# simochen/flowtrack.pytorch

Hardware: AMD Instinct MI355X
Metric: pose crops/sec (ResNet-50 + 3-deconv head, 256x192) (higher is better)
Workload: dtype fp16; 1 GPU; ResNet-50 pose head fp16, batch 64 x 256x192 synthetic crops per GPU (BASELINE.json configs[1]); per_gpu_batch=64, resident_batches=4, parallelism=dp1: batch sharded, one process per GPU

## Files before the change

### flowtrack/pytorch_amd/_lib.py

```python
from __future__ import annotations

import ctypes
import os
from ctypes import POINTER, c_char_p, c_double, c_float, c_int, c_int32, c_uint64, c_void_p

HERE = os.path.dirname(os.path.abspath(__file__))
LIB_PATH = os.environ.get("FT_LIB_PATH") or os.path.join(HERE, "libflowtrack_hip.so")

FT_OK = 0
FT_ERR_INVALID_ARG = 1
FT_ERR_UNSUPPORTED = 2
FT_F16, FT_F32 = 0, 1
FT_ACT_NONE, FT_ACT_RELU, FT_ACT_LEAKY = 0, 1, 2
FT_LAYOUT_NHWC, FT_LAYOUT_NCHW_F32 = 0, 1
FT_RGB_MEAN_SPLITS = 64
FT_BNK_Y_FULL, FT_BNK_Y_EVEN, FT_BNK_Y_NONE = 0, 1, 2


class FlowtrackHipError(RuntimeError):
    pass


class ConvDesc(ctypes.Structure):

# ... 43 lines not shown
    "ft_stream_synchronize": (c_int, [c_void_p]),
    "ft_memcpy_async": (c_int, [c_void_p, c_void_p, ctypes.c_size_t, c_void_p]),
    "ft_conv_pack_geometry": (c_int, [POINTER(ConvDesc), POINTER(ConvGeometry)]),
    "ft_conv_tile_candidates": (c_int, [POINTER(ConvDesc), POINTER(c_int), c_int]),
    "ft_conv_workspace_bytes": (ctypes.c_size_t, [POINTER(ConvDesc)]),
    "ft_conv2d_fwd_ws": (c_int, [POINTER(ConvDesc), c_void_p, c_void_p, c_void_p, c_void_p, c_void_p, c_void_p, c_void_p,
                                 ctypes.c_size_t, c_void_p]),
    "ft_conv_tap_source": (c_int, [POINTER(ConvDesc), c_int, c_int, c_int, POINTER(c_int), POINTER(c_int)]),
    "ft_conv2d_fwd": (c_int, [POINTER(ConvDesc), c_void_p, c_void_p, c_void_p, c_void_p, c_void_p,
                              c_void_p, c_void_p]),
    "ft_conv_flops": (c_double, [POINTER(ConvDesc)]),
    "ft_conv_direct_supported": (c_int, [POINTER(ConvDesc)]),
    "ft_conv_direct_stream_id": (c_int, [POINTER(ConvDesc)]),
    "ft_conv_direct_weight_bytes": (ctypes.c_longlong, [POINTER(ConvDesc)]),
    "ft_conv_direct_pack": (c_int, [POINTER(ConvDesc), c_void_p, c_int, c_int, c_void_p, c_void_p]),
    "ft_conv_direct_fwd": (c_int, [POINTER(ConvDesc), c_void_p, c_void_p, c_void_p, c_void_p, c_void_p, c_void_p, c_void_p]),
    "ft_bottleneck_supported": (c_int, [POINTER(BottleneckDesc)]),
    "ft_bottleneck_fwd": (c_int, [POINTER(BottleneckDesc), c_void_p, c_void_p, c_void_p, c_void_p, c_void_p, c_void_p, c_void_p]),
    "ft_bottleneck_flops": (c_double, [POINTER(BottleneckDesc)]),
    "ft_bottleneck_exit_supported": (c_int, [POINTER(BottleneckDesc), c_int, c_int, c_int, c_int]),
    "ft_bottleneck_exit_weight_bytes": (ctypes.c_longlong, [POINTER(BottleneckDesc), c_int]),
    "ft_bottleneck_exit_pack": (c_int, [POINTER(BottleneckDesc), c_int, c_void_p, c_int, c_int, c_void_p, c_void_p]),
    "ft_bottleneck_exit_fwd": (c_int, [POINTER(BottleneckDesc), c_void_p, c_void_p, c_void_p, c_void_p, c_void_p, c_void_p, c_int, c_int,
                                       c_void_p, c_void_p, c_void_p, c_void_p, c_int, c_int, c_void_p]),
    "ft_bottleneck_rstat_supported": (c_int, [POINTER(BottleneckDesc)]),
    "ft_bottleneck_rstat_weight_bytes": (ctypes.c_longlong, []),
    "ft_bottleneck_rstat_fwd": (c_int, [POINTER(BottleneckDesc), c_void_p, c_void_p, c_void_p, c_void_p]),
    "ft_bottleneck_stream_supported": (c_int, [POINTER(BottleneckDesc)]),
    "ft_bottleneck_stream_folds": (c_int, [POINTER(BottleneckDesc)]),
    "ft_bottleneck_stream_layout": (c_int, [POINTER(BottleneckDesc)]),
    "ft_bottleneck_stream_weight_bytes": (ctypes.c_longlong, [POINTER(BottleneckDesc)]),
    "ft_bottleneck_stream_pack": (c_int, [POINTER(BottleneckDesc), c_void_p, c_void_p, c_void_p, c_void_p, c_void_p]),
    "ft_bottleneck_stream_fwd": (c_int, [POINTER(BottleneckDesc), c_void_p, c_void_p, c_void_p, c_void_p, c_void_p]),
    "ft_pack_nchw_to_nhwc": (c_int, [c_void_p, c_void_p] + [c_int] * 8 + [c_void_p]),
    "ft_unpack_nhwc_to_nchw": (c_int, [c_void_p, c_void_p, c_int, c_int, c_int, c_int, c_int, c_int, c_int,
                                       c_void_p]),
    "ft_maxpool3x3s2_fwd": (c_int, [c_void_p, c_void_p, c_int, c_int, c_int, c_int, c_int, c_void_p]),
    "ft_bn_batch_stats": (c_int, [c_void_p, c_int, c_int, c_int, c_int, c_int, c_int, c_void_p, c_void_p, c_void_p, c_void_p]),
    "ft_heatmap_max_preds": (c_int, [c_void_p, c_int, c_int, c_int, c_int, c_int, c_void_p, c_void_p, c_void_p,
                                     c_void_p]),
    "ft_heatmap_keypoint_rows": (c_int, [c_void_p, c_int, c_int, c_int, c_int, c_int, c_void_p, c_void_p, c_void_p]),
    "ft_heatmap_min_margin": (c_int, [c_void_p, c_int, c_int, c_int, c_int, c_void_p, c_void_p]),
    "ft_heatmap_argmax_screen": (c_int, [c_void_p, c_int, c_int, c_int, c_int, c_float, c_void_p, c_void_p, c_void_p]),
    "ft_flow_rgb_mean": (c_int, [c_void_p, c_int, c_int, c_int, c_void_p, c_void_p, c_void_p]),
    "ft_flow_pack_pair": (c_int, [c_void_p, c_void_p, c_float, c_void_p] + [c_int] * 7 + [c_void_p]),
    "ft_flow_mean_pack_pair_state_words": (ctypes.c_longlong, [c_int, c_int, c_int]),
    "ft_flow_pack_pair_sums_chunks": (ctypes.c_longlong, [c_int]),
    "ft_conv_shift_nstride_supported": (c_int, [POINTER(ConvDesc)]),
    "ft_flow_pack_pair_sums": (c_int, [c_void_p, c_float, c_void_p] + [c_int] * 6 + [c_void_p, c_void_p]),
    "ft_flow_mean_fold": (c_int, [c_void_p, c_float, c_void_p] + [c_int] * 6 + [c_void_p, c_void_p, c_void_p, c_int, c_void_p, c_void_p,
                                  c_void_p]),
    "ft_flow_mean_pack_pair": (c_int, [c_void_p, c_float, c_void_p, c_int, c_int, c_void_p, c_int, c_int] + [c_int] * 4
                               + [c_void_p, c_void_p, c_void_p]),
    "ft_upsample_bilinear4x": (c_int, [c_void_p, c_void_p, c_int, c_int, c_int, c_int, c_float, c_void_p]),
    "ft_correlation_out_shape": (c_int, [c_int] * 8 + [POINTER(c_int)] * 3),
    "ft_correlation_fwd": (c_int, [c_void_p, c_void_p, c_void_p] + [c_int] * 10 + [c_void_p]),
    "ft_correlation_nhwc_fwd": (c_int, [c_void_p, c_void_p, c_void_p] + [c_int] * 10 + [c_float, c_int, c_void_p]),
    "ft_resample2d_fwd": (c_int, [c_void_p, c_void_p, c_void_p, c_int, c_int, c_int, c_int, c_void_p]),
    "ft_channelnorm_fwd": (c_int, [c_void_p, c_void_p, c_int, c_int, c_int, c_int, c_void_p]),
    "ft_correlation_bwd": (c_int, [c_void_p] * 5 + [c_int] * 10 + [c_void_p]),
    "ft_resample2d_bwd": (c_int, [c_void_p] * 5 + [c_int] * 4 + [c_void_p]),
    "ft_channelnorm_bwd": (c_int, [c_void_p] * 4 + [c_int] * 4 + [c_void_p]),
    "ft_upsample_nearest4x": (c_int, [c_void_p, c_void_p, c_int, c_int, c_int, c_int, c_float, c_void_p]),
    "ft_flow_fusion_concat": (c_int, [c_void_p, c_void_p, c_void_p, c_void_p] + [c_int] * 8 + [c_void_p]),
    "ft_crop_affine_fwd": (c_int, [c_void_p, c_int, c_int, c_int, c_void_p, c_int, c_int, c_int, c_void_p, c_void_p, c_float,
                                   c_void_p, c_void_p]),
# ... 52 lines not shown
```

### flowtrack/pytorch_amd/csrc/bottleneck_stream.hip

```cpp
#include <stdlib.h>

#include <type_traits>

#include "ft_common.h"

namespace ft {
namespace {

struct BnsParams {
  const char* x;
  char* y;
  const char* ws;
  const char* tab;
  int H, W, TH;
  int ppi, total;
  int TWc, csplit;
  int Ho, Wo;
  int x_cstride, x_coff, y_cstride, y_coff;
  unsigned x_bytes, y_bytes, ws_bytes;
  int dbg;
};

template <int N, int I = 0, typename F>
__device__ __forceinline__ void bns_unroll(F&& f) {
// ... 1849 lines not shown
  if (pl.variant == 4) { p.Ho = d->H / 2; p.Wo = d->W / 2; }
  p.total = d->N * pl.ppi;
  p.x_cstride = d->x_cstride; p.x_coff = d->x_coff; p.y_cstride = d->y_cstride; p.y_coff = d->y_coff;
  p.x_bytes = (unsigned)((size_t)d->N * d->H * d->W * d->x_cstride * 2);
  p.y_bytes = (unsigned)((size_t)d->N * d->H * d->W * d->y_cstride * 2);
  p.ws_bytes = (unsigned)ft_bottleneck_stream_weight_bytes(d);
  if (pl.variant == 4) p.y_bytes = (unsigned)((size_t)d->N * p.Ho * p.Wo * d->y_cstride * 2);
  static const int dbg = dev_env_int("FT_BNS_DBG", 0);
  p.dbg = dbg;
  if (dbg & 64) p.ws_bytes = 0;
  if (dbg & 128) p.x_bytes = 0;
  hipStream_t s = as_stream(stream);
  const bool waves8 = dev_env_int("FT_BNS_WAVES", pl.variant == 3 ? 8 : 4) == 8;
  if (d->folded) {
    switch (pl.variant) {
      case 0: return bns_launch<128, 4, 3, true>(p, s);
      case 5: return bns_launch<128, 3, 2, true>(p, s);
      case 1: return bns_launch<256, 4, 3, true>(p, s);
      case 6: return bns_launch_tile16(p, s);
      case 3: return waves8 ? bns_launch_direct<2, 1, true, 0, 8, true>(p, s) : bns_launch_direct<2, 1, true, 0, 4, true>(p, s);
      default: return waves8 ? bns_launch_direct<3, 2, false, 0, 8, true>(p, s) : bns_launch_direct<3, 2, false, 0, 4, true>(p, s);
    }
  }
  switch (pl.variant) {
    case 0: return bns_launch<128, 4, 3>(p, s);
    case 5: return bns_launch<128, 3, 2>(p, s);
    case 1: return bns_launch<256, 4, 3>(p, s);
    case 3: return waves8 ? bns_launch_direct<2, 1, true, 0, 8>(p, s) : bns_launch_direct<2, 1, true>(p, s);
    case 4: return waves8 ? bns_launch_direct<4, 1, false, 8, 8>(p, s) : bns_launch_direct<4, 1, false, 8>(p, s);
    default:
      return waves8 ? bns_launch_direct<3, 2, false, 0, 8>(p, s) : bns_launch_direct<3, 2, false>(p, s);
  }
}
```

### flowtrack/pytorch_amd/hip_ops.py

```python
from __future__ import annotations

import ctypes
import functools
import json
import os
import sys
from dataclasses import dataclass
from typing import List, Optional, Sequence, Tuple

import torch

from . import _lib
from ._lib import (FT_ACT_LEAKY, FT_ACT_NONE, FT_ACT_RELU, FT_LAYOUT_NCHW_F32, FT_LAYOUT_NHWC,
                   ConvDesc, ConvGeometry, FlowtrackHipError, check)

ACT_CODES = {None: FT_ACT_NONE, "none": FT_ACT_NONE, "relu": FT_ACT_RELU, "leaky": FT_ACT_LEAKY}


def require_gpu(device: torch.device) -> None:
    if device.type != "cuda" or not torch.cuda.is_available():
        raise FlowtrackHipError(
            "the flowtrack HIP path needs a ROCm GPU (model.cuda()); there is no CPU fallback — "
            "use oracle/ for CPU reference results")

# ... 13 lines not shown
    @property
    def N(self): return self.t.shape[0]
    @property
    def H(self): return self.t.shape[1]
    @property
    def W(self): return self.width if self.width is not None else self.t.shape[2]
    @property
    def wpitch(self): return self.t.shape[2]
    @property
    def rowpacked(self): return self.width is not None
    @property
    def cstride(self): return self.t.shape[3]

    def batch_slice(self, lo: int, hi: int) -> "ActView":
        return ActView(self.t[lo:hi], self.C, self.coff, self.lpad, self.width)


def act_stride(C: int) -> int:
    return round_up(C, 32) if C >= 32 else round_up(C, 8)


def new_rowpacked_act(N: int, H: int, W: int, C: int, pad: int, dtype, device) -> ActView:
    cpad = 4 if C <= 4 else round_up(C, 8)
    wpitch = round_up(W + 2 * pad, 2)
    return ActView(torch.zeros((N, H, wpitch, cpad), dtype=dtype, device=device), C, 0, pad, W)


def new_act(N: int, H: int, W: int, C: int, dtype, device, cstride: Optional[int] = None) -> ActView:
    cs = act_stride(C) if cstride is None else cstride
    return ActView(torch.zeros((N, H, W, cs), dtype=dtype, device=device), C, 0)


def is_conv_call(name: str) -> bool:
    return name.startswith("ft_conv2d_fwd") or name in ("ft_bottleneck_fwd", "ft_bottleneck_exit_fwd", "ft_bottleneck_rstat_fwd", "ft_bottleneck_stream_fwd", "ft_bottleneck_cluster_fwd", "ft_conv_direct_fwd")


def _on_plan_device(fn):
    @functools.wraps(fn)
    def wrapper(self, *args, **kwargs):
        if self.stream is None:
            return fn(self, *args, **kwargs)
        with torch.cuda.device(self.stream.device):
            return fn(self, *args, **kwargs)
    return wrapper


class Program:

    def __init__(self, stream: torch.cuda.Stream):
        self.lib = _lib.load()
        self.stream = stream
        self.calls: List[Tuple[str, tuple]] = []
        self.lanes: List[int] = []
        self.keepalive: list = []
        self.graph_exec = None
        self.flops = 0.0
        self.conv_records: list = []
        self.fused_records: list = []
        self._ws_ptr, self._ws_size = ctypes.c_void_p(None), ctypes.c_size_t(0)
        self._ws_need, self._ws_tensor = 0, None
        self._side = False
        self._side_stream: Optional[torch.cuda.Stream] = None
        self._choice_flops: list = []
        self._events: list = []

    @property
    def stream_handle(self) -> ctypes.c_void_p:
# ... 1120 lines not shown
    args = _bottleneck_exit_args(x, y, t1, c2.cin, y_mode)
    if args is None:
        raise FlowtrackHipError(f"{label}: views do not fit y mode {y_mode!r}")
    d, mode = args
    def overlap(a, b):
        a0, b0 = a.t.data_ptr(), b.t.data_ptr()
        return a0 < b0 + b.t.numel() * b.t.element_size() and b0 < a0 + a.t.numel() * a.t.element_size()
    if overlap(t1, x) or (y is not None and (overlap(y, x) or overlap(t1, y))):
        raise FlowtrackHipError(f"{label}: x, y and t1 of the exit form must be three separate buffers")
    planes = c2.cin
    check(lib.ft_bottleneck_exit_supported(ctypes.byref(d), tail.cout, t1.cstride, t1.coff, mode), "ft_bottleneck_exit_supported")
    w1, s1, b1 = _bottleneck_packed(c1, x, (planes, x.C, 1), label)
    w2, s2, b2 = _bottleneck_packed(c2, x, (planes, 9 * planes, 1), label)
    w3, s3, b3 = _bottleneck_packed(c3, x, (x.C, planes, 1), label)
    wt, st, bt = _bottleneck_packed(tail, x, (tail.cout, x.C, 1), label)
    key = ("bnk_exit", wt.data_ptr())
    wstream = tail._packed.get(key)
    if wstream is None:
        wstream = torch.empty(int(lib.ft_bottleneck_exit_weight_bytes(ctypes.byref(d), tail.cout)), dtype=torch.uint8, device=x.t.device)
        check(lib.ft_bottleneck_exit_pack(ctypes.byref(d), tail.cout, wt.data_ptr(), int(wt.shape[-1]), int(wt.shape[-2]), wstream.data_ptr(),
                                          current_stream_handle(x.t.device)), "ft_bottleneck_exit_pack")
        torch.cuda.current_stream(x.t.device).synchronize()
        tail._packed[key] = wstream
    table = torch.cat([t.flatten()[:n] for t, n in ((s1, planes), (b1, planes), (s2, planes), (b2, planes), (s3, x.C), (b3, x.C))]).contiguous()
    tscale, tshift = st.flatten()[:tail.cout].contiguous(), bt.flatten()[:tail.cout].contiguous()
    flops = float(lib.ft_bottleneck_flops(ctypes.byref(d))) + 2.0 * x.N * x.H * x.W * x.C * tail.cout
    prog.flops += flops
    prog.fused_records.append((label, len(prog.calls), flops))
    prog.add("ft_bottleneck_exit_fwd", ctypes.byref(d), x.t.data_ptr(), w1.data_ptr(), w2.data_ptr(), w3.data_ptr(), table.data_ptr(),
             y.t.data_ptr() if y is not None else None, mode, tail.cout, wstream.data_ptr(), tscale.data_ptr(), tshift.data_ptr(),
             t1.t.data_ptr(), t1.cstride, t1.coff, keep=(d, x.t, y.t if y is not None else None, t1.t, w1, w2, w3, table, wstream, tscale, tshift))


def record_pack_input(prog: Program, x_nchw: torch.Tensor, y: ActView) -> None:
    N, C, H, W = x_nchw.shape
    prog.add("ft_pack_nchw_to_nhwc", x_nchw.data_ptr(), y.t.data_ptr(), N, C, H, W, y.cstride, y.lpad, y.wpitch,
             _lib.dtype_code(y.t.dtype), keep=(x_nchw, y.t))


def record_maxpool(prog: Program, x: ActView, y: ActView) -> None:
    if x.coff or y.coff or x.cstride != x.C or y.cstride != y.C:
        raise FlowtrackHipError("maxpool works on dense NHWC buffers")
    prog.add("ft_maxpool3x3s2_fwd", x.t.data_ptr(), y.t.data_ptr(), x.N, x.H, x.W, x.C, _lib.dtype_code(x.t.dtype),
             keep=(x.t, y.t))


def record_upsample4x(prog: Program, x: torch.Tensor, y: torch.Tensor, mul: float) -> None:
    N, C, h, w = x.shape
    prog.add("ft_upsample_bilinear4x", x.data_ptr(), y.data_ptr(), N, C, h, w, ctypes.c_float(mul), keep=(x, y))


def current_stream_handle(device=None) -> ctypes.c_void_p:
    return ctypes.c_void_p(torch.cuda.current_stream(device).cuda_stream)


def heatmap_max_preds(heatmaps: torch.Tensor, adjust_coords: bool):
    require_gpu(heatmaps.device)
    lib = _lib.load()
    hm = heatmaps.contiguous().float()
    N, K, H, W = hm.shape
    idx = torch.empty((N, K), dtype=torch.int32, device=hm.device)
    score = torch.empty((N, K, 1), dtype=torch.float32, device=hm.device)
    coords = torch.empty((N, K, 2), dtype=torch.float32, device=hm.device)
    check(lib.ft_heatmap_max_preds(hm.data_ptr(), N, K, H, W, int(bool(adjust_coords)), idx.data_ptr(),
                                   score.data_ptr(), coords.data_ptr(), current_stream_handle()),
          "ft_heatmap_max_preds")
# ... 16 lines not shown
```

### flowtrack/pytorch_amd/pose/models.py

```python
from __future__ import annotations

import math
import os
from typing import List

import torch
import torch.nn as nn

from ..engine import HipModule
from ..hip_ops import (ActView, FlowtrackHipError, FusedConv, FusedShortcutConv, Program, bottleneck_exit_fusable, bottleneck_fusable,
                       bottleneck_entry_fusable, bottleneck_head_fusable, bottleneck_cluster_supported, bottleneck_strips_supported, bottleneck_head_stream_fusable, bottleneck_prefers_fused, new_act, new_rowpacked_act, record_bottleneck, record_bottleneck_entry, record_bottleneck_head, record_bottleneck_head_stream,
                       record_bottleneck_exit, record_maxpool, record_pack_input)
from ..params import ActMarker, BatchNormParams, ConvParams, ConvTransposeParams

resnet_dict = {50: [3, 4, 6, 3], 101: [3, 4, 23, 3], 152: [3, 8, 36, 3]}


class Bottleneck(nn.Module):
    expansion = 4

    def __init__(self, inplanes: int, planes: int, stride: int = 1):
        super().__init__()
        self.stride = stride
        self.conv1 = ConvParams(inplanes, planes, 1, bias=False)
        self.bn1 = BatchNormParams(planes)
        self.conv2 = ConvParams(planes, planes, 3, stride=stride, padding=1, bias=False)
        self.bn2 = BatchNormParams(planes)
        self.conv3 = ConvParams(planes, planes * 4, 1, bias=False)
        self.bn3 = BatchNormParams(planes * 4)
        self.relu = ActMarker("relu")
        if stride != 1 or inplanes != planes * 4:
            self.downsample = nn.Sequential(ConvParams(inplanes, planes * 4, 1, stride=stride, bias=False),
                                            BatchNormParams(planes * 4))
        else:
            self.downsample = nn.Sequential()


class _PosePlan:
    def __init__(self, prog, x_static, heatmaps):
        self.prog, self.x_static, self.heatmaps = prog, x_static, heatmaps
        self.runs = 0


class _Stages(dict):

    def __init__(self, *a, **k):
        super().__init__(*a, **k)
        self.absent = {}

    def __missing__(self, key):
        if key in self.absent:
            raise FlowtrackHipError(f"plan.stages[{key!r}]: {self.absent[key]}")
        raise KeyError(key)


class DeconvResnet(HipModule):
    fuse_shortcut: bool = os.environ.get("FT_FUSE_SHORTCUT", "1") != "0"
    fuse_bottleneck: bool = os.environ.get("FT_FUSE_BOTTLENECK", "1") != "0"
    fuse_stage_exit = {"0": False, "2": "force"}.get(os.environ.get("FT_FUSE_STAGE_EXIT", "1"), True)
    fuse_stem_pool: bool = os.environ.get("FT_FUSE_STEM_POOL", "1") != "0"
    fuse_stem_pack: bool = os.environ.get("FT_FUSE_STEM_PACK", "1") != "0"
    keypoints_in_plan = None
    exact_in_plan: bool = False
    split_lanes4: bool = os.environ.get("FT_SPLIT_LANES4", "0") == "1"
    split_lanes: int = int(os.environ.get("FT_SPLIT_LANES", "0") or 0)
    fuse_heatmap: bool = os.environ.get("FT_FUSE_HEATMAP", "1") != "0"
    exact_argmax_rel_bound: float = 1.6e-3

    def __init__(self, layers: List[int], num_classes: int):
        super().__init__()
        self.layers_cfg = list(layers)
        self.num_classes = num_classes
        self.inplanes = 64
        self.conv1 = ConvParams(3, 64, 7, stride=2, padding=3, bias=False)
        self.bn1 = BatchNormParams(64)
        self.relu = ActMarker("relu")
        self.maxpool = ActMarker("maxpool3x3s2")
        self.layer1 = self._make_layer(64, layers[0])
        self.layer2 = self._make_layer(128, layers[1], stride=2)
        self.layer3 = self._make_layer(256, layers[2], stride=2)
        self.layer4 = self._make_layer(512, layers[3], stride=2)
        self.deconv_bias = False
        feats = 256
        self.deconv = nn.Sequential(
            ConvTransposeParams(2048, feats, bias=False), BatchNormParams(feats), ActMarker("relu"),
            ConvTransposeParams(feats, feats, bias=False), BatchNormParams(feats), ActMarker("relu"),
            ConvTransposeParams(feats, feats, bias=False), BatchNormParams(feats), ActMarker("relu"))
        self.heatmap = ConvParams(feats, num_classes, 1, bias=True)

    def _make_layer(self, planes: int, blocks: int, stride: int = 1) -> nn.Sequential:
        mods = [Bottleneck(self.inplanes, planes, stride)]
        self.inplanes = planes * 4
# ... 164 lines not shown
                prog.add("ft_gather_flagged_rows", ex["flags"].data_ptr(), B, x_static.data_ptr(), ctypes.c_longlong(3 * H * W * 4), ex["stage"].data_ptr(),
                         ex["header"].data_ptr(), keep=(ex["stage"], ex["header"]))
                prog.add("ft_memcpy_async", ex["header_host"].data_ptr(), ex["header"].data_ptr(), ctypes.c_size_t((1 + B) * 4), keep=(ex["header_host"],))
                plan.exact = ex
        return plan

    def _record_stage_exit(self, prog, name: str, blk, nname: str, nblk, cur, out, dtype, device):
        if not (self.fuse_stage_exit and self.fuse_bottleneck and self.fuse_shortcut) or dtype != torch.float16:
            return None
        if len(blk.downsample) or blk.stride != 1 or nblk.stride != 2 or not len(nblk.downsample) or cur.H % 2 or cur.W % 2:
            return None
        B, mk = cur.N, dict(dtype=dtype, device=device)
        nplanes = nblk.conv1.cout
        c1 = self.fused(name + ".conv1", blk.conv1.weight, bn=blk.bn1.as_dict(), act="relu", **mk)
        c2 = self.fused(name + ".conv2", blk.conv2.weight, stride=1, pad=1, bn=blk.bn2.as_dict(), act="relu", **mk)
        c3 = self.fused(name + ".conv3", blk.conv3.weight, bn=blk.bn3.as_dict(), act="relu", **mk)
        n1 = self.fused(nname + ".conv1", nblk.conv1.weight, bn=nblk.bn1.as_dict(), act="relu", **mk)
        n2 = self.fused(nname + ".conv2", nblk.conv2.weight, stride=2, pad=1, bn=nblk.bn2.as_dict(), act="relu", **mk)
        t1 = new_act(B, cur.H, cur.W, nplanes, dtype, device)
        y_even = new_act(B, cur.H // 2, cur.W // 2, cur.C, dtype, device)
        if not bottleneck_exit_fusable(c1, c2, c3, n1, cur, y_even, t1, "even"):
            return None
        t2 = new_act(B, cur.H // 2, cur.W // 2, nplanes, dtype, device)
        nout = new_act(B, cur.H // 2, cur.W // 2, nplanes * 4, dtype, device)
        key = (nname + ".conv3+downsample@even", dtype, str(device))
        sc = self._layers.get(key)
        if sc is None:
            sc = self._layers[key] = FusedShortcutConv(nblk.conv3.weight, nblk.bn3.as_dict(), nblk.downsample[0].weight,
                                                       nblk.downsample[1].as_dict(), 1, dtype=dtype, device=device, act="relu",
                                                       label=nname + ".conv3+downsample")

        def exit_form():
            record_bottleneck_exit(prog, c1, c2, c3, n1, cur, y_even, t1, f"{name}.fused+{nname}.conv1", "even")
            n2.record(prog, t1, t2)
            sc.record(prog, t2, y_even, nout)

        def block_form():
            self._record_block(prog, name, blk, cur, out, dtype, device)
            self._record_block(prog, nname, nblk, out, nout, dtype, device)
        if self.fuse_stage_exit == "force":
            exit_form()
            return nout
        prog.begin_choice(f"bottleneck|exit,{B},{cur.H},{cur.W},{cur.C},{nplanes},{cur.cstride}")
        for form_name, form in (("fused", exit_form), ("convs", block_form)):
            prog.option(form_name)
            form()
        prog.end_choice()
        return nout

    def _record_block(self, prog, name: str, blk, cur, out, dtype, device) -> None:
        B = cur.N
        mk = dict(dtype=dtype, device=device)
        planes = blk.conv1.cout
        s = blk.stride
        Ho, Wo = cur.H // s, cur.W // s
        c1 = self.fused(name + ".conv1", blk.conv1.weight, bn=blk.bn1.as_dict(), act="relu", **mk)
        c2 = self.fused(name + ".conv2", blk.conv2.weight, stride=s, pad=1, bn=blk.bn2.as_dict(), act="relu", **mk)
        c3 = self.fused(name + ".conv3", blk.conv3.weight, bn=blk.bn3.as_dict(), act="relu", **mk)
        if self.fuse_bottleneck and not len(blk.downsample) and s == 1 and bottleneck_fusable(c1, c2, c3, cur, out):
            t1 = new_act(B, cur.H, cur.W, planes, dtype, device)
            t2 = new_act(B, Ho, Wo, planes, dtype, device)

            def fused_form():
                record_bottleneck(prog, c1, c2, c3, cur, out, name + ".fused", form="patch")

            def conv_form():
                c1.record(prog, cur, t1)
                c2.record(prog, t1, t2)
# ... 332 lines not shown
```

### include/flowtrack_hip.h

```cpp
#ifndef FLOWTRACK_HIP_H_
#define FLOWTRACK_HIP_H_

#include <stddef.h>
#include <stdint.h>

#ifdef __cplusplus
extern "C" {
#endif

enum {
  FT_OK = 0,
  FT_ERR_INVALID_ARG = 1,
  FT_ERR_UNSUPPORTED = 2,
  FT_ERR_HIP = 3,
  FT_ERR_NO_DEVICE = 4
};

enum { FT_F16 = 0, FT_F32 = 1 };
enum { FT_ACT_NONE = 0, FT_ACT_RELU = 1, FT_ACT_LEAKY = 2 };
enum { FT_LAYOUT_NHWC = 0, FT_LAYOUT_NCHW_F32 = 1 };

typedef void* ft_stream_t;

int ft_version(void);
// ... 77 lines not shown
  int C, P;
  int x_cstride, x_coff;
  int y_cstride, y_coff;
  int head_only;
  int projection;
  int stride;
  int folded;
} ft_bottleneck_desc;
int ft_bottleneck_supported(const ft_bottleneck_desc* d);
int ft_bottleneck_fwd(const ft_bottleneck_desc* d, const void* x,
                      const void* w1, const void* w2, const void* w3,
                      const float* scale_shift, void* y, ft_stream_t stream);
double ft_bottleneck_flops(const ft_bottleneck_desc* d);

enum { FT_BNK_Y_FULL = 0, FT_BNK_Y_EVEN = 1, FT_BNK_Y_NONE = 2 };
int ft_bottleneck_exit_supported(const ft_bottleneck_desc* d, int tail_cout, int t1_cstride, int t1_coff, int y_mode);
long long ft_bottleneck_exit_weight_bytes(const ft_bottleneck_desc* d, int tail_cout);
int ft_bottleneck_exit_pack(const ft_bottleneck_desc* d, int tail_cout, const void* wt_packed, int kpad, int cout_pad, void* wstream,
                            ft_stream_t stream);
int ft_bottleneck_exit_fwd(const ft_bottleneck_desc* d, const void* x, const void* w1, const void* w2, const void* w3,
                           const float* scale_shift, void* y, int y_mode, int tail_cout, const void* tail_wstream,
                           const float* tail_scale, const float* tail_shift, void* t1, int t1_cstride, int t1_coff,
                           ft_stream_t stream);

int ft_bottleneck_stream_supported(const ft_bottleneck_desc* d);
int ft_bottleneck_stream_folds(const ft_bottleneck_desc* d);
int ft_bottleneck_stream_layout(const ft_bottleneck_desc* d);
long long ft_bottleneck_stream_weight_bytes(const ft_bottleneck_desc* d);
int ft_bottleneck_stream_pack(const ft_bottleneck_desc* d, const void* w1, const void* w2, const void* w3, void* wstream,
                              ft_stream_t stream);
int ft_bottleneck_stream_fwd(const ft_bottleneck_desc* d, const void* x, const void* wstream, const float* tables, void* y,
                             ft_stream_t stream);

int ft_pack_nchw_to_nhwc(const float* x, void* y, int N, int C, int H, int W,
                         int cpad, int lpad, int wpitch, int dtype,
                         ft_stream_t stream);
int ft_unpack_nhwc_to_nchw(const void* x, float* y, int N, int C, int H, int W,
                           int x_cstride, int x_coff, int dtype,
                           ft_stream_t stream);
int ft_maxpool3x3s2_fwd(const void* x, void* y, int N, int Hi, int Wi, int C,
                        int dtype, ft_stream_t stream);

int ft_bn_batch_stats(const void* x, int N, int H, int W, int C, int x_cstride, int dtype,
                      float* workspace, float* mean, float* var, ft_stream_t stream);

int ft_heatmap_max_preds(const float* heatmaps, int N, int K, int H, int W,
                         int adjust_coords, int32_t* idx, float* score,
                         float* coords, ft_stream_t stream);
int ft_heatmap_keypoint_rows(const float* heatmaps, int N, int K, int H, int W,
                             int adjust_coords, int32_t* idx, float* rows,
                             ft_stream_t stream);

int ft_heatmap_min_margin(const float* heatmaps, int N, int K, int H, int W, float* min_margin, ft_stream_t stream);

int ft_heatmap_argmax_screen(const float* heatmaps, int N, int K, int H, int W, float rel_bound, int32_t* flags, float* stats,
                             ft_stream_t stream);

int ft_gather_flagged_rows(const int32_t* flags, int N, const void* src, long long row_bytes, void* dst, int32_t* header,
                           ft_stream_t stream);

#define FT_RGB_MEAN_SPLITS 64
int ft_flow_rgb_mean(const float* inputs, int B, int H, int W, float* partial,
                     float* mean, ft_stream_t stream);
int ft_flow_pack_pair(const float* inputs, const float* mean, float rgb_max,
                      void* y, int B, int H, int W, int mode, int lpad,
                      int wpitch, int dtype, ft_stream_t stream);
// ... 83 lines not shown
```

Before: 59150 crops/s.

## Fuse stage-entry bottleneck tail (strided 3x3 conv + shortcut conv) into one kernel

Adds a HIP kernel that runs the stride-2 3x3 conv2 with BN+ReLU and feeds its output through LDS directly into the fused conv3+downsample shortcut GEMM, writing the block output once. It is meant to remove the intermediate t2 activation round-trip through global memory and one kernel launch at the stage-entry blocks (P=128). The kernel streams packed weights through a triple-buffered LDS pipeline and uses buffer-to-LDS loads. It is registered as a tunable choice against the existing two-conv path, so the planner can fall back if it is not better. The cost is a large, specialised kernel that only covers one geometry.

```diff
diff --git a/flowtrack/pytorch_amd/_lib.py b/flowtrack/pytorch_amd/_lib.py
--- a/flowtrack/pytorch_amd/_lib.py
+++ b/flowtrack/pytorch_amd/_lib.py
@@ -99,6 +99,11 @@
     "ft_bottleneck_stream_weight_bytes": (ctypes.c_longlong, [POINTER(BottleneckDesc)]),
     "ft_bottleneck_stream_pack": (c_int, [POINTER(BottleneckDesc), c_void_p, c_void_p, c_void_p, c_void_p, c_void_p]),
     "ft_bottleneck_stream_fwd": (c_int, [POINTER(BottleneckDesc), c_void_p, c_void_p, c_void_p, c_void_p, c_void_p]),
+    "ft_bottleneck_tail_supported": (c_int, [POINTER(BottleneckDesc), c_int, c_int, c_int, c_int]),
+    "ft_bottleneck_tail_weight_bytes": (ctypes.c_longlong, [POINTER(BottleneckDesc)]),
+    "ft_bottleneck_tail_pack": (c_int, [POINTER(BottleneckDesc), c_void_p, c_int, c_void_p, c_int, c_int, c_void_p, c_void_p]),
+    "ft_bottleneck_tail_fwd": (c_int, [POINTER(BottleneckDesc), c_void_p, c_void_p, c_void_p, c_void_p, c_int, c_int, c_int, c_int, c_void_p,
+                                       c_void_p]),
     "ft_pack_nchw_to_nhwc": (c_int, [c_void_p, c_void_p] + [c_int] * 8 + [c_void_p]),
     "ft_unpack_nhwc_to_nchw": (c_int, [c_void_p, c_void_p, c_int, c_int, c_int, c_int, c_int, c_int, c_int,
                                        c_void_p]),
diff --git a/flowtrack/pytorch_amd/csrc/bottleneck_stream.hip b/flowtrack/pytorch_amd/csrc/bottleneck_stream.hip
--- a/flowtrack/pytorch_amd/csrc/bottleneck_stream.hip
+++ b/flowtrack/pytorch_amd/csrc/bottleneck_stream.hip
@@ -1905,3 +1905,438 @@
       return waves8 ? bns_launch_direct<3, 2, false, 0, 8>(p, s) : bns_launch_direct<3, 2, false>(p, s);
   }
 }
+
+namespace ft {
+namespace {
+
+struct BnsTailParams {
+  const char* t1;
+  const char* ye;
+  char* y;
+  const char* ws;
+  const char* tab;
+  int H, W, Ho, Wo, TH;
+  int ppi, total;
+  int x_cstride, x_coff, ye_cstride, ye_coff, y_cstride, y_coff;
+  unsigned x_bytes, ye_bytes, y_bytes, ws_bytes;
+  int dbg;
+};
+
+struct BnsTailGeom {
+  static constexpr int P = 128, NCT = 4, KC = 2, WSTEP = NCT * 4096, LW = NCT, ROWB = 256, MT = 3, NOUT = 96;
+  static constexpr int YKC = 4;
+  static constexpr int G3 = 9 * KC, QSTEPS = KC + YKC, GEND = G3 + 4 * QSTEPS;
+  static constexpr int PATCH_ROWS = 432, NPIECE = PATCH_ROWS / 4;
+  static constexpr int YB = NOUT * ROWB, YCH = NOUT * 128, STG = YB + YKC * YCH;
+  static constexpr int TAB = PATCH_ROWS * ROWB, TABB = 8 * P, ZROW = TAB + TABB, SCR = ZROW + 1024;
+  static constexpr int WBASE = 114688, LDS_BYTES = 163840;
+  static_assert(MT * 32 == NOUT && LW * 4096 == WSTEP, "4 x 1 waves: one channel tile x MT pixel tiles, LW 1-KiB loads per wave and step");
+  static_assert(NPIECE % 4 == 0 && STG + NOUT * ROWB <= TAB && SCR + 1024 <= WBASE && WBASE + 3 * WSTEP == LDS_BYTES && ZROW % ROWB == 0, "LDS map");
+};
+
+__global__ __launch_bounds__(256, 1) void bottleneck_tail_kernel(const BnsTailParams p) {
+#if defined(__HIP_DEVICE_COMPILE__)
+  using G = BnsTailGeom;
+  constexpr int P = G::P, NCT = G::NCT, KC = G::KC, WSTEP = G::WSTEP, LW = G::LW, ROWB = G::ROWB, MT = G::MT;
+  constexpr int LP = G::NPIECE / 4;
+  constexpr int LY = G::YKC * G::YCH / 4096;
+  constexpr int kTouch = 6;
+  static_assert(LP + 3 * LW + 1 + kTouch <= 63, "vmcnt immediate");
+  extern __shared__ __attribute__((aligned(16))) char smem[];
+  typedef __attribute__((address_space(3))) void* lds_ptr;
+  using c0 = std::integral_constant<int, 0>;
+  using c1 = std::integral_constant<int, 1>;
+  const int tid = threadIdx.x, lane = tid & 63;
+  const int wave = __builtin_amdgcn_readfirstlane(tid >> 6);
+  const int l31 = lane & 31, lhi = lane >> 5;
+
+  int logical;
+  {
+    const int b = blockIdx.x;
+    const int q = p.total >> 3, r = p.total & 7, xcd = b & 7, loc = b >> 3;
+    logical = (xcd < r ? xcd * (q + 1) : r * (q + 1) + (xcd - r) * q) + loc;
+  }
+  const int n = logical / p.ppi;
+  const int y0 = (logical - n * p.ppi) * p.TH;
+  const int W = p.W, Wo = p.Wo;
+  const int rows_out = p.Ho - y0 < p.TH ? p.Ho - y0 : p.TH;
+  const int npix_out = rows_out * Wo;
+  const int npatch = (2 * p.TH + 1) * W;
+  const int opix0 = (n * p.Ho + y0) * Wo;
+
+  const __amdgpu_buffer_rsrc_t rsrc_x = __builtin_amdgcn_make_buffer_rsrc(const_cast<char*>(p.t1), 0, p.x_bytes, 0x00020000);
+  const __amdgpu_buffer_rsrc_t rsrc_e = __builtin_amdgcn_make_buffer_rsrc(const_cast<char*>(p.ye), 0, p.ye_bytes, 0x00020000);
+  const __amdgpu_buffer_rsrc_t rsrc_y = __builtin_amdgcn_make_buffer_rsrc(p.y, 0, p.y_bytes, 0x00020000);
+  const __amdgpu_buffer_rsrc_t rsrc_w = __builtin_amdgcn_make_buffer_rsrc(const_cast<char*>(p.ws), 0, p.ws_bytes, 0x00020000);
+  const __amdgpu_buffer_rsrc_t rsrc_t = __builtin_amdgcn_make_buffer_rsrc(const_cast<char*>(p.tab), 0, 5 * G::TABB, 0x00020000);
+  constexpr unsigned kOOB = 0x80000000u;
+  const unsigned lane16 = (unsigned)lane * 16u;
+
+  auto issue_patch = [&]() {
+#pragma unroll
+    for (int t = 0; t < LP; ++t) {
+      const int piece = t * 4 + wave;
+      const int row = piece * 4 + (lane >> 4);
+      const int pr = row / W, pc = row - pr * W;
+      const int iy = 2 * y0 - 1 + pr;
+      unsigned v = kOOB;
+      if (row < npatch && (unsigned)iy < (unsigned)p.H)
+        v = (unsigned)((((n * p.H + iy) * W + pc) * p.x_cstride + p.x_coff) * 2 + (((lane & 15) ^ ((row >> 1) & 15)) << 4));
+      __builtin_amdgcn_raw_ptr_buffer_load_lds(rsrc_x, (lds_ptr)(smem + piece * 1024), 16, v, 0, 0, 0);
+    }
+  };
+  auto issue_y = [&]() {
+#pragma unroll
+    for (int t = 0; t < LY; ++t) {
+      const int piece = t * 4 + wave;
+      const int c = piece / (G::YCH / 1024), r8 = piece - c * (G::YCH / 1024);
+      const int m = r8 * 8 + (lane >> 3);
+      const unsigned v = m < npix_out ? (unsigned)(((opix0 + m) * p.ye_cstride + p.ye_coff) * 2 + (((lane & 7) ^ BNS_XKEY(m)) << 4)) : kOOB;
+      __builtin_amdgcn_raw_ptr_buffer_load_lds(rsrc_e, (lds_ptr)(smem + G::YB + piece * 1024), 16, v, c * 128, 0, 0);
+    }
+  };
+  auto issue_w = [&](int g, int buf) {
+    char* dst = smem + G::WBASE + buf * WSTEP;
+#pragma unroll
+    for (int t = 0; t < LW; ++t)
+      __builtin_amdgcn_raw_ptr_buffer_load_lds(rsrc_w, (lds_ptr)(dst + (t * 4 + wave) * 1024), 16, lane16, g * WSTEP + (t * 4 + wave) * 1024, 0, 0);
+  };
+  auto issue_tab = [&](int e) {
+    __builtin_amdgcn_raw_ptr_buffer_load_lds(rsrc_t, (lds_ptr)(smem + G::TAB + wave * 256), 4, (unsigned)lane * 4u, e * G::TABB + wave * 256, 0, 0);
+  };
+  auto issue_touch = [&]() {
+    const bool on = blockIdx.x < 256 && !(p.dbg & (512 | 1024));
+    const int xcd = blockIdx.x & 7, loc = blockIdx.x >> 3;
+    const int first = p.total < 256 ? p.total : 256;
+    const int nloc = (first - xcd + 7) >> 3;
+    const unsigned lines = (p.ws_bytes + 127u) >> 7;
+    const unsigned per = (lines + nloc - 1) / nloc;
+    const unsigned lo = loc * per, hi = lo + per < lines ? lo + per : lines;
+#pragma unroll
+    for (int k = 0; k < kTouch; ++k) {
+      const unsigned l = lo + tid + 256u * k;
+      __builtin_amdgcn_raw_ptr_buffer_load_lds(rsrc_w, (lds_ptr)(smem + G::SCR + wave * 256), 4, (on && l < hi) ? l << 7 : kOOB, 0, 0, 0);
+    }
+  };
+
+  unsigned long long ts[8] = {0, 0, 0, 0, 0, 0, 0, 0};
+#define BNT_TS(i) do { if (p.dbg & 32) ts[i] = __builtin_amdgcn_s_memtime(); } while (0)
+  BNT_TS(0);
+  issue_patch();
+  issue_w(0, 0);
+  issue_tab(0);
+  issue_touch();
+  asm volatile("" ::: "memory");
+  issue_w(1, 1);
+  issue_w(2, 2);
+  if (tid < ROWB / 16) *reinterpret_cast<uint4_t*>(smem + G::ZROW + tid * 16) = uint4_t{0u, 0u, 0u, 0u};
+
+  int m_out[MT], pbase[MT], edge[MT];
+#pragma unroll
+  for (int j = 0; j < MT; ++j) {
+    m_out[j] = j * 32 + l31;
+    const int mc = m_out[j] < npix_out ? m_out[j] : 0;
+    const int r = mc / Wo, c = mc - r * Wo;
+    pbase[j] = 2 * r * W + 2 * c - 1;
+    edge[j] = c == 0;
+  }
+
+  const unsigned a_base = (unsigned)(G::WBASE + wave * 1024) + lane16;
+  uint4_t fa[4];
+  uint4_t fb[4][MT];
+  float16_t acc[MT];
+  auto zero_acc = [&]() {
+#pragma unroll
+    for (int j = 0; j < MT; ++j)
+#pragma unroll
+      for (int r = 0; r < 16; ++r) acc[j][r] = 0.f;
+  };
+  zero_acc();
+  auto ld = [&](auto kkc, int buf, const int (&rb)[MT]) {
+    constexpr int kk = decltype(kkc)::value;
+    fa[kk] = *reinterpret_cast<const uint4_t*>(smem + a_base + buf * WSTEP + kk * NCT * 1024);
+#pragma unroll
+    for (int j = 0; j < MT; ++j) fb[kk][j] = *reinterpret_cast<const uint4_t*>(smem + (rb[j] ^ (kk << 5)));
+  };
+  auto mma = [&](auto kkc) {
+    constexpr int kk = decltype(kkc)::value;
+#pragma unroll
+    for (int j = 0; j < MT; ++j)
+      acc[j] = __builtin_amdgcn_mfma_f32_32x32x16_f16(__builtin_bit_cast(half8_t, fa[kk]), __builtin_bit_cast(half8_t, fb[kk][j]), acc[j], 0, 0, 0);
+  };
+  auto bases_patch = [&](int off, int kc, bool left, int (&rb)[MT]) {
+#pragma unroll
+    for (int j = 0; j < MT; ++j) {
+      const int row = pbase[j] + off;
+      const int v = row * ROWB + ((((row >> 1) & 15) ^ lhi) << 4);
+      rb[j] = ((left && edge[j]) ? G::ZROW + (lhi << 4) : v) ^ (kc << 7);
+    }
+  };
+  auto bases_c = [&](int ks, int (&rb)[MT]) {
+#pragma unroll
+    for (int j = 0; j < MT; ++j) {
+      const int m = m_out[j];
+      rb[j] = ks < KC ? (m * ROWB + (((m & 15) ^ lhi) << 4)) ^ (ks << 7)
+                      : G::YB + (ks - KC) * G::YCH + m * 128 + ((lhi ^ BNS_XKEY(m)) << 4);
+    }
+  };
+  using c2 = std::integral_constant<int, 2>;
+  using c3 = std::integral_constant<int, 3>;
+  auto pstep = [&](int g, int buf, const int (&rb)[MT], bool has_next, const int (&rb_next)[MT], int tab_e, auto waitc) {
+    __builtin_amdgcn_sched_barrier(0);
+    ld(c2{}, buf, rb);
+    __builtin_amdgcn_sched_barrier(0);
+    mma(c0{});
+    __builtin_amdgcn_sched_barrier(0);
+    ld(c3{}, buf, rb);
+    __builtin_amdgcn_sched_barrier(0);
+    mma(c1{});
+    __builtin_amdgcn_sched_barrier(0);
+    if (has_next) {
+      asm volatile("s_waitcnt vmcnt(%0) lgkmcnt(0)" ::"n"(decltype(waitc)::value) : "memory");
+      BNS_BARRIER();
+      if (tab_e >= 0) issue_tab(tab_e);
+      if (g + 3 < G::GEND) issue_w(g + 3, buf);
+      ld(c0{}, buf == 2 ? 0 : buf + 1, rb_next);
+      __builtin_amdgcn_sched_barrier(0);
+    }
+    mma(c2{});
+    __builtin_amdgcn_sched_barrier(0);
+    if (has_next) {
+      ld(c1{}, buf == 2 ? 0 : buf + 1, rb_next);
+      __builtin_amdgcn_sched_barrier(0);
+    }
+    mma(c3{});
+  };
+  using wLW = std::integral_constant<int, LW>;
+
+  {
+    int rb[MT], rbn[MT];
+    bases_patch(0, 0, true, rb);
+    asm volatile("s_waitcnt vmcnt(%0) lgkmcnt(0)" ::"n"(2 * LW) : "memory");
+    BNS_BARRIER();
+    BNT_TS(1);
+    ld(c0{}, 0, rb);
+    ld(c1{}, 0, rb);
+    int g = 0, buf = 0;
+    for (int tap = 0; tap < 9; ++tap) {
+      const int ky = tap / 3, kx = tap - 3 * ky;
+#pragma unroll
+      for (int kc = 0; kc < KC; ++kc) {
+        const bool has_next = !(tap == 8 && kc == KC - 1);
+        int nky = ky, nkx = kx, nkc = kc + 1;
+        if (nkc == KC) { nkc = 0; if (++nkx == 3) { nkx = 0; ++nky; } }
+        bases_patch(nky * W + nkx, nkc, nkx == 0, rbn);
+        pstep(g, buf, rb, has_next, rbn, -1, wLW{});
+#pragma unroll
+        for (int j = 0; j < MT; ++j) rb[j] = rbn[j];
+        ++g;
+        buf = buf == 2 ? 0 : buf + 1;
+      }
+    }
+  }
+  BNT_TS(2);
+  asm volatile("s_waitcnt lgkmcnt(0)" ::: "memory");
+  BNS_BARRIER();
+  issue_y();
+  const float* tb = reinterpret_cast<const float*>(smem + G::TAB);
+  const int ch = wave * 32 + 16 * lhi;
+  {
+    float4_t sc[4], sh[4];
+#pragma unroll
+    for (int g4 = 0; g4 < 4; ++g4) {
+      sc[g4] = *reinterpret_cast<const float4_t*>(tb + ch + g4 * 4);
+      sh[g4] = *reinterpret_cast<const float4_t*>(tb + P + ch + g4 * 4);
+    }
+#pragma unroll
+    for (int j = 0; j < MT; ++j) {
+      const int m = m_out[j];
+      half8_t h8[2];
+      bn_relu_acc16(acc[j], sc, sh, h8);
+      char* rowp = smem + m * ROWB;
+      const int cb = wave * 4 + 2 * lhi;
+#pragma unroll
+      for (int h = 0; h < 2; ++h) *reinterpret_cast<half8_t*>(rowp + (((cb + h) ^ (m & 15)) << 4)) = h8[h];
+    }
+  }
+  zero_acc();
+
+  {
+    constexpr int CPR = ROWB / 16;
+    constexpr int NSTG = G::NOUT * CPR / 256;
+    unsigned s_voff[NSTG];
+    int s_off[NSTG];
+#pragma unroll
+    for (int k = 0; k < NSTG; ++k) {
+      const int idx = tid + 256 * k, m = idx / CPR, cc = idx % CPR;
+      s_voff[k] = m < npix_out ? (unsigned)(((opix0 + m) * p.y_cstride + p.y_coff + cc * 8) * 2) : kOOB;
+      s_off[k] = G::STG + m * ROWB + ((cc ^ (m & 15)) << 4);
+    }
+    int rb[MT];
+    bases_c(0, rb);
+    asm volatile("s_waitcnt vmcnt(%0) lgkmcnt(0)" ::"n"(LW + LY) : "memory");
+    BNS_BARRIER();
+    BNT_TS(3);
+    issue_tab(1);
+    issue_w(G::G3 + 2, (G::G3 + 2) % 3);
+    ld(c0{}, G::G3 % 3, rb);
+    ld(c1{}, G::G3 % 3, rb);
+    bns_unroll<4>([&](auto qc) {
+      constexpr int q = decltype(qc)::value;
+      bns_unroll<G::QSTEPS>([&](auto ksc) {
+        constexpr int ks = decltype(ksc)::value;
+        constexpr int g = G::G3 + q * G::QSTEPS + ks;
+        int rbn[MT];
+        bases_c(ks + 1 < G::QSTEPS ? ks + 1 : 0, rbn);
+        constexpr int wait_n = g == G::G3 ? LY + 1 + LW : (g + 2 < G::GEND ? LW : 0);
+        pstep(g, g % 3, rb, g + 1 < G::GEND, rbn, (ks == 0 && q > 0) ? 1 + q : -1, std::integral_constant<int, wait_n>{});
+#pragma unroll
+        for (int j = 0; j < MT; ++j) rb[j] = rbn[j];
+      });
+      if constexpr (q == 3) {
+        asm volatile("s_waitcnt vmcnt(0)" ::: "memory");
+        BNS_BARRIER();
+      }
+      float4_t sc[4], sh[4];
+#pragma unroll
+      for (int g4 = 0; g4 < 4; ++g4) {
+        sc[g4] = *reinterpret_cast<const float4_t*>(tb + ch + g4 * 4);
+        sh[g4] = *reinterpret_cast<const float4_t*>(tb + P + ch + g4 * 4);
+      }
+#pragma unroll
+      for (int j = 0; j < MT; ++j) {
+        const int m = m_out[j];
+        half8_t o8[2];
+        bn_relu_acc16(acc[j], sc, sh, o8);
+#pragma unroll
+        for (int h = 0; h < 2; ++h)
+          *reinterpret_cast<half8_t*>(smem + G::STG + m * ROWB + (((wave * 4 + 2 * lhi + h) ^ (m & 15)) << 4)) = o8[h];
+      }
+      zero_acc();
+      asm volatile("s_waitcnt lgkmcnt(0)" ::: "memory");
+      BNS_BARRIER();
+#pragma unroll
+      for (int k = 0; k < NSTG; ++k) {
+        const uint4_t v = *reinterpret_cast<const uint4_t*>(smem + s_off[k]);
+        if (!(p.dbg & 4)) __builtin_amdgcn_raw_buffer_store_b128(v, rsrc_y, s_voff[k] + (unsigned)(q * P * 2), 0, FT_YSTORE_BUF_AUX);
+      }
+    });
+  }
+  if (p.dbg & 32) {
+    ts[4] = __builtin_amdgcn_s_memtime();
+    asm volatile("s_waitcnt vmcnt(0)" ::: "memory");
+    ts[5] = __builtin_amdgcn_s_memtime();
+    if (tid == 0) {
+      unsigned long long* o = reinterpret_cast<unsigned long long*>(p.y + ((size_t)opix0 * p.y_cstride + p.y_coff) * 2);
+#pragma unroll
+      for (int i = 0; i < 8; ++i) o[i] = ts[i];
+    }
+  }
+#endif
+}
+
+__global__ __launch_bounds__(256) void bns_pack_tail_kernel(const half_t* __restrict__ w2, int kpad2, const half_t* __restrict__ w3d, int kpad3,
+                                                            int koff_d, uint4_t* __restrict__ out) {
+  using G = BnsTailGeom;
+  const int idx = blockIdx.x * 256 + threadIdx.x;
+  if (idx >= G::GEND * G::WSTEP / 16) return;
+  const int lane = idx & 63, frag = idx >> 6;
+  const int per_step = 4 * G::NCT;
+  const int g = frag / per_step, f = frag - g * per_step;
+  const int kk = f / G::NCT, i = f - kk * G::NCT;
+  const int l31 = lane & 31, lhi = lane >> 5;
+  const int co_t = 32 * i + bns_sigma(l31);
+  const int k_t = 16 * kk + 8 * lhi;
+  const half_t* src;
+  if (g < G::G3) {
+    const int tap = g / G::KC, kc = g - tap * G::KC;
+    src = w2 + (size_t)co_t * kpad2 + tap * G::P + 64 * kc + k_t;
+  } else {
+    const int s = g - G::G3, q = s / G::QSTEPS, ks = s - q * G::QSTEPS;
+    const int k = ks < G::KC ? 64 * ks : koff_d + 64 * (ks - G::KC);
+    src = w3d + (size_t)(q * G::P + co_t) * kpad3 + k + k_t;
+  }
+  out[idx] = *reinterpret_cast<const uint4_t*>(src);
+}
+
+struct BnsTailPlan { int TH, ppi; };
+
+static int bns_tail_plan(const ft_bottleneck_desc* d, int ye_h, int ye_w, int ye_cstride, int ye_coff, BnsTailPlan* out) {
+  using G = BnsTailGeom;
+  if (!d) return FT_ERR_INVALID_ARG;
+  if (d->N <= 0 || d->H <= 0 || d->W <= 0) return FT_ERR_INVALID_ARG;
+  if (d->dtype != FT_F16 || d->P != G::P || d->C != 4 * G::P || d->stride != 2 || !d->projection || d->head_only || d->folded) return FT_ERR_UNSUPPORTED;
+  if ((d->H & 1) || (d->W & 1)) return FT_ERR_UNSUPPORTED;
+  const int Ho = d->H / 2, Wo = d->W / 2;
+  if (ye_h != Ho || ye_w != Wo) return FT_ERR_UNSUPPORTED;
+  if (d->x_coff < 0 || d->y_coff < 0 || ye_coff < 0 || d->x_coff % 8 || d->y_coff % 8 || ye_coff % 8 || d->x_cstride % 8 || d->y_cstride % 8 || ye_cstride % 8)
+    return FT_ERR_UNSUPPORTED;
+  if (d->x_cstride < d->x_coff + d->P || d->y_cstride < d->y_coff + d->C || ye_cstride < ye_coff + 2 * d->P) return FT_ERR_UNSUPPORTED;
+  if ((long long)d->N * d->H * d->W * d->x_cstride * 2 >= (1LL << 31) || (long long)d->N * Ho * Wo * d->y_cstride * 2 >= (1LL << 31) ||
+      (long long)d->N * Ho * Wo * ye_cstride * 2 >= (1LL << 31))
+    return FT_ERR_UNSUPPORTED;
+  int th = G::NOUT / Wo;
+  const int th2 = (G::PATCH_ROWS / d->W - 1) / 2;
+  th = th < th2 ? th : th2;
+  if (th < 1) return FT_ERR_UNSUPPORTED;
+  th = th < Ho ? th : Ho;
+  th = ceil_div(Ho, ceil_div(Ho, th));
+  if (out) *out = BnsTailPlan{th, ceil_div(Ho, th)};
+  return FT_OK;
+}
+
+}
+}
+
+extern "C" int ft_bottleneck_tail_supported(const ft_bottleneck_desc* d, int ye_h, int ye_w, int ye_cstride, int ye_coff) {
+  return ft::bns_tail_plan(d, ye_h, ye_w, ye_cstride, ye_coff, nullptr);
+}
+
+extern "C" long long ft_bottleneck_tail_weight_bytes(const ft_bottleneck_desc* d) {
+  if (!d || d->dtype != FT_F16 || d->P != ft::BnsTailGeom::P || d->C != 4 * d->P) return 0;
+  return (long long)ft::BnsTailGeom::GEND * ft::BnsTailGeom::WSTEP;
+}
+
+extern "C" int ft_bottleneck_tail_pack(const ft_bottleneck_desc* d, const void* w2_packed, int kpad2, const void* w3d_packed, int kpad3, int koff_d,
+                                       void* wstream, ft_stream_t stream) {
+  using namespace ft;
+  using G = BnsTailGeom;
+  if (ft_bottleneck_tail_weight_bytes(d) == 0) return d ? FT_ERR_UNSUPPORTED : FT_ERR_INVALID_ARG;
+  if (!w2_packed || !w3d_packed || !wstream) return FT_ERR_INVALID_ARG;
+  if (kpad2 < 9 * G::P || kpad2 % 8 || koff_d < G::P || koff_d % 8 || kpad3 < koff_d + 2 * G::P || kpad3 % 8) return FT_ERR_INVALID_ARG;
+  const int n16 = G::GEND * G::WSTEP / 16;
+  hipLaunchKernelGGL(bns_pack_tail_kernel, dim3(ceil_div(n16, 256)), dim3(256), 0, as_stream(stream), static_cast<const half_t*>(w2_packed), kpad2,
+                     static_cast<const half_t*>(w3d_packed), kpad3, koff_d, static_cast<uint4_t*>(wstream));
+  FT_LAUNCH_CHECK("bns_pack_tail_kernel");
+  return FT_OK;
+}
+
+extern "C" int ft_bottleneck_tail_fwd(const ft_bottleneck_desc* d, const void* t1, const void* wstream, const float* tables, const void* y_even,
+                                      int ye_h, int ye_w, int ye_cstride, int ye_coff, void* out, ft_stream_t stream) {
+  using namespace ft;
+  BnsTailPlan pl;
+  const int st = bns_tail_plan(d, ye_h, ye_w, ye_cstride, ye_coff, &pl);
+  if (st != FT_OK) return st;
+  if (!t1 || !wstream || !tables || !y_even || !out || out == t1 || out == y_even) return FT_ERR_INVALID_ARG;
+  BnsTailParams p{};
+  p.t1 = static_cast<const char*>(t1);
+  p.ye = static_cast<const char*>(y_even);
+  p.y = static_cast<char*>(out);
+  p.ws = static_cast<const char*>(wstream);
+  p.tab = reinterpret_cast<const char*>(tables);
+  p.H = d->H; p.W = d->W; p.Ho = d->H / 2; p.Wo = d->W / 2; p.TH = pl.TH; p.ppi = pl.ppi;
+  p.total = d->N * pl.ppi;
+  p.x_cstride = d->x_cstride; p.x_coff = d->x_coff; p.ye_cstride = ye_cstride; p.ye_coff = ye_coff; p.y_cstride = d->y_cstride; p.y_coff = d->y_coff;
+  p.x_bytes = (unsigned)((size_t)d->N * d->H * d->W * d->x_cstride * 2);
+  p.ye_bytes = (unsigned)((size_t)d->N * p.Ho * p.Wo * ye_cstride * 2);
+  p.y_bytes = (unsigned)((size_t)d->N * p.Ho * p.Wo * d->y_cstride * 2);
+  p.ws_bytes = (unsigned)ft_bottleneck_tail_weight_bytes(d);
+  static const int dbg = dev_env_int("FT_BNS_DBG", 0);
+  p.dbg = dbg;
+  if (dbg & 64) p.ws_bytes = 0;
+  if (dbg & 128) p.x_bytes = p.ye_bytes = 0;
+  FT_RAISE_LDS(bottleneck_tail_kernel, BnsTailGeom::LDS_BYTES);
+  hipLaunchKernelGGL(bottleneck_tail_kernel, dim3(p.total), dim3(256), BnsTailGeom::LDS_BYTES, as_stream(stream), p);
+  FT_LAUNCH_CHECK("bottleneck_tail_kernel");
+  return FT_OK;
+}
diff --git a/flowtrack/pytorch_amd/hip_ops.py b/flowtrack/pytorch_amd/hip_ops.py
--- a/flowtrack/pytorch_amd/hip_ops.py
+++ b/flowtrack/pytorch_amd/hip_ops.py
@@ -69,7 +69,7 @@
 
 
 def is_conv_call(name: str) -> bool:
-    return name.startswith("ft_conv2d_fwd") or name in ("ft_bottleneck_fwd", "ft_bottleneck_exit_fwd", "ft_bottleneck_rstat_fwd", "ft_bottleneck_stream_fwd", "ft_bottleneck_cluster_fwd", "ft_conv_direct_fwd")
+    return name.startswith("ft_conv2d_fwd") or name in ("ft_bottleneck_fwd", "ft_bottleneck_exit_fwd", "ft_bottleneck_rstat_fwd", "ft_bottleneck_stream_fwd", "ft_bottleneck_cluster_fwd", "ft_bottleneck_tail_fwd", "ft_conv_direct_fwd")
 
 
 def _on_plan_device(fn):
@@ -1256,6 +1256,68 @@
              t1.t.data_ptr(), t1.cstride, t1.coff, keep=(d, x.t, y.t if y is not None else None, t1.t, w1, w2, w3, table, wstream, tscale, tshift))
 
 
+def _bottleneck_tail_args(c2: "FusedConv", sc: "FusedShortcutConv", t1: ActView, y_even: ActView, out: ActView):
+    if not isinstance(sc, FusedShortcutConv) or t1.t.dtype != torch.float16 or t1.rowpacked or y_even.rowpacked or out.rowpacked:
+        return None
+    if y_even.t.dtype != t1.t.dtype or out.t.dtype != t1.t.dtype or (y_even.N, out.N) != (t1.N, t1.N):
+        return None
+    if (c2.k, c2.stride, c2.pad, c2.cin, c2.cout) != (3, 2, 1, t1.C, t1.C) or c2.transposed or c2.tail_cout or c2.act != ACT_CODES["relu"] \
+            or c2._bn is None:
+        return None
+    if (sc.cin, sc.cin2, sc.cout, sc.stride_d) != (t1.C, y_even.C, out.C, 1) or sc.act != ACT_CODES["relu"]:
+        return None
+    if (out.H, out.W) != (t1.H // 2, t1.W // 2) or y_even.C != 2 * t1.C or out.C != 4 * t1.C:
+        return None
+    d = _lib.BottleneckDesc()
+    d.dtype = _lib.dtype_code(t1.t.dtype)
+    d.N, d.H, d.W, d.C, d.P = t1.N, t1.H, t1.W, out.C, t1.C
+    d.x_cstride, d.x_coff, d.y_cstride, d.y_coff = t1.cstride, t1.coff, out.cstride, out.coff
+    d.stride, d.projection = 2, 1
+    return d
+
+
+def bottleneck_tail_fusable(c2: "FusedConv", sc: "FusedShortcutConv", t1: ActView, y_even: ActView, out: ActView) -> bool:
+    d = _bottleneck_tail_args(c2, sc, t1, y_even, out)
+    if d is None:
+        return False
+    return _lib.load().ft_bottleneck_tail_supported(ctypes.byref(d), y_even.H, y_even.W, y_even.cstride, y_even.coff) == 0
+
+
+def record_bottleneck_tail(prog: Program, c2: "FusedConv", sc: "FusedShortcutConv", t1: ActView, y_even: ActView, out: ActView,
+                           label: str) -> None:
+    lib = _lib.load()
+    d = _bottleneck_tail_args(c2, sc, t1, y_even, out)
+    if d is None:
+        raise FlowtrackHipError(f"{label}: layers / views are not a stage-entry tail")
+    ye = (y_even.H, y_even.W, y_even.cstride, y_even.coff)
+    check(lib.ft_bottleneck_tail_supported(ctypes.byref(d), *ye), "ft_bottleneck_tail_supported")
+    for a, b in ((out, t1), (out, y_even)):
+        a0, b0 = a.t.data_ptr(), b.t.data_ptr()
+        if a0 < b0 + b.t.numel() * b.t.element_size() and b0 < a0 + a.t.numel() * a.t.element_size():
+            raise FlowtrackHipError(f"{label}: the tail's output must not share a buffer with its inputs")
+    P = c2.cin
+    w2, s2, b2 = _bottleneck_packed(c2, t1, (P, 9 * P, 1), label)
+    key = ("bns_tail", w2.data_ptr())
+    cached = sc._packed.get(key)
+    if cached is None:
+        dev = t1.t.device
+        w3d = torch.cat([sc._w3, sc._wd], dim=1).to(device=dev, dtype=torch.float16).contiguous()
+        shift = sc._shift.float()
+        tables = torch.cat([s2.flatten()[:P].float().cpu(), b2.flatten()[:P].float().cpu()] +
+                           [t for q in range(4) for t in (torch.ones(P), shift[q * P:(q + 1) * P])]).contiguous().to(dev)
+        wstream = torch.empty(int(lib.ft_bottleneck_tail_weight_bytes(ctypes.byref(d))), dtype=torch.uint8, device=dev)
+        check(lib.ft_bottleneck_tail_pack(ctypes.byref(d), w2.data_ptr(), int(w2.shape[-1]), w3d.data_ptr(), int(w3d.shape[-1]), P,
+                                          wstream.data_ptr(), current_stream_handle(dev)), "ft_bottleneck_tail_pack")
+        torch.cuda.current_stream(dev).synchronize()
+        cached = sc._packed[key] = (wstream, tables)
+    wstream, tables = cached
+    flops = 2.0 * out.N * out.H * out.W * (P * 9 * P + out.C * (P + y_even.C))
+    prog.flops += flops
+    prog.fused_records.append((label, len(prog.calls), flops))
+    prog.add("ft_bottleneck_tail_fwd", ctypes.byref(d), t1.t.data_ptr(), wstream.data_ptr(), tables.data_ptr(), y_even.t.data_ptr(), *ye,
+             out.t.data_ptr(), keep=(d, t1.t, y_even.t, out.t, wstream, tables))
+
+
 def record_pack_input(prog: Program, x_nchw: torch.Tensor, y: ActView) -> None:
     N, C, H, W = x_nchw.shape
     prog.add("ft_pack_nchw_to_nhwc", x_nchw.data_ptr(), y.t.data_ptr(), N, C, H, W, y.cstride, y.lpad, y.wpitch,
diff --git a/flowtrack/pytorch_amd/pose/models.py b/flowtrack/pytorch_amd/pose/models.py
--- a/flowtrack/pytorch_amd/pose/models.py
+++ b/flowtrack/pytorch_amd/pose/models.py
@@ -9,6 +9,7 @@
 
 from ..engine import HipModule
 from ..hip_ops import (ActView, FlowtrackHipError, FusedConv, FusedShortcutConv, Program, bottleneck_exit_fusable, bottleneck_fusable,
+                       bottleneck_tail_fusable, record_bottleneck_tail,
                        bottleneck_entry_fusable, bottleneck_head_fusable, bottleneck_cluster_supported, bottleneck_strips_supported, bottleneck_head_stream_fusable, bottleneck_prefers_fused, new_act, new_rowpacked_act, record_bottleneck, record_bottleneck_entry, record_bottleneck_head, record_bottleneck_head_stream,
                        record_bottleneck_exit, record_maxpool, record_pack_input)
 from ..params import ActMarker, BatchNormParams, ConvParams, ConvTransposeParams
@@ -58,6 +59,7 @@
     fuse_shortcut: bool = os.environ.get("FT_FUSE_SHORTCUT", "1") != "0"
     fuse_bottleneck: bool = os.environ.get("FT_FUSE_BOTTLENECK", "1") != "0"
     fuse_stage_exit = {"0": False, "2": "force"}.get(os.environ.get("FT_FUSE_STAGE_EXIT", "1"), True)
+    fuse_stage_tail = {"0": False, "2": "force"}.get(os.environ.get("FT_FUSE_STAGE_TAIL", "1"), True)
     fuse_stem_pool: bool = os.environ.get("FT_FUSE_STEM_POOL", "1") != "0"
     fuse_stem_pack: bool = os.environ.get("FT_FUSE_STEM_PACK", "1") != "0"
     keypoints_in_plan = None
@@ -288,8 +290,23 @@
 
         def exit_form():
             record_bottleneck_exit(prog, c1, c2, c3, n1, cur, y_even, t1, f"{name}.fused+{nname}.conv1", "even")
-            n2.record(prog, t1, t2)
-            sc.record(prog, t2, y_even, nout)
+
+            def tail_convs():
+                n2.record(prog, t1, t2)
+                sc.record(prog, t2, y_even, nout)
+
+            def tail_fused():
+                record_bottleneck_tail(prog, n2, sc, t1, y_even, nout, f"{nname}.tail")
+            if not (self.fuse_stage_tail and bottleneck_tail_fusable(n2, sc, t1, y_even, nout)):
+                tail_convs()
+            elif self.fuse_stage_tail == "force":
+                tail_fused()
+            else:
+                prog.begin_choice(f"bottleneck|tail,{B},{cur.H},{cur.W},{nplanes},{t1.cstride},{y_even.cstride},{nout.cstride}")
+                for form_name, form in (("convs", tail_convs), ("fused", tail_fused)):
+                    prog.option(form_name)
+                    form()
+                prog.end_choice()
 
         def block_form():
             self._record_block(prog, name, blk, cur, out, dtype, device)
diff --git a/include/flowtrack_hip.h b/include/flowtrack_hip.h
--- a/include/flowtrack_hip.h
+++ b/include/flowtrack_hip.h
@@ -133,6 +133,13 @@
 int ft_bottleneck_stream_fwd(const ft_bottleneck_desc* d, const void* x, const void* wstream, const float* tables, void* y,
                              ft_stream_t stream);
 
+int ft_bottleneck_tail_supported(const ft_bottleneck_desc* d, int ye_h, int ye_w, int ye_cstride, int ye_coff);
+long long ft_bottleneck_tail_weight_bytes(const ft_bottleneck_desc* d);
+int ft_bottleneck_tail_pack(const ft_bottleneck_desc* d, const void* w2_packed, int kpad2, const void* w3d_packed, int kpad3, int koff_d,
+                            void* wstream, ft_stream_t stream);
+int ft_bottleneck_tail_fwd(const ft_bottleneck_desc* d, const void* t1, const void* wstream, const float* tables, const void* y_even,
+                           int ye_h, int ye_w, int ye_cstride, int ye_coff, void* out, ft_stream_t stream);
+
 int ft_pack_nchw_to_nhwc(const float* x, void* y, int N, int C, int H, int W,
                          int cpad, int lpad, int wpitch, int dtype,
                          ft_stream_t stream);
```

Measured after the change: 59400 crops/s (median of 6 runs). Within noise of the previous version (+0.4%).
